# luvk1412/RoaringBitmap

Measured on AMD Instinct MI355X. Metric: wide-OR/pairwise-AND input GB/s + % of HBM peak at 1/2/4/8 MI355X, higher is better.
Workload: dtype u64; 1 GPU; C2: RoaringBitmap.and(x1, x2), two full 2^32-universe bitmaps of 65536 mixed array/bitmap/run containers each (configs[1]); per_rank=the whole pair, parallelism=key-range sharding over 1 GPU(s)

## Files before the change

### roaringbitmap_amd/csrc/pairwise.hip

```cpp
#include <algorithm>
#include <cstdio>
#include <cstdlib>

#include "kernels.hpp"
#include "wave.hpp"

namespace rbg {

__device__ __forceinline__ int pair_class(int op, int ka, int kb) {
  if (ka == kAbsent || kb == kAbsent) return 1;
  if (op == OP_AND && (ka == DK_A || kb == DK_A)) return 1;
  if (op == OP_ANDNOT && ka == DK_A) return 1;
  return 2;
}

__global__ __launch_bounds__(256) void k_plan_pairwise(int op, int key_lo, int key_hi, const uint32_t* __restrict__ koa,
                                                       const CDesc* __restrict__ da, const uint8_t* __restrict__ pa,
                                                       const uint32_t* __restrict__ kob,
                                                       const CDesc* __restrict__ db, const uint8_t* __restrict__ pb,
                                                       uint64_t* __restrict__ wg_epoch, uint32_t epoch,
                                                       PTask* __restrict__ tasks, uint32_t* __restrict__ n_tasks,
                                                       uint64_t* zlb, uint64_t* ztile, uint32_t* err) {
  plan_zero(zlb, ztile);
  const uint32_t k = blockIdx.x * blockDim.x + threadIdx.x;
// ... 37 lines not shown
    c = 18 + n / 300;
  }
  return kBalBins - 1 - min(c, kBalBins - 1);
}

template <int OP, int MODE>
__global__ __launch_bounds__(256) void k_plan_balanced(int key_lo, uint32_t nkeys, const uint32_t* __restrict__ koa,
                                                       const CDesc* __restrict__ da, const uint8_t* __restrict__ pa,
                                                       const uint32_t* __restrict__ kob,
                                                       const CDesc* __restrict__ db, const uint8_t* __restrict__ pb,
                                                       PTask* __restrict__ tasks, uint32_t* __restrict__ n_tasks,
                                                       OutCtx oc, uint32_t* __restrict__ task_card, uint64_t* zlb,
                                                       uint64_t* ztile) {
  __shared__ int hist[kBalBins];
  __shared__ int off[kBalBins];
  plan_zero(zlb, ztile);
  if (threadIdx.x < kBalBins) hist[threadIdx.x] = 0;
  __syncthreads();
  const uint32_t i = blockIdx.x * blockDim.x + threadIdx.x;
  PTask t;
  int bin = kBalBins - 1, rank = 0;
  if (i < nkeys) {
    const uint32_t k = (uint32_t)key_lo + i;
    resolve(koa, da, pa, k, t.slot_a, t.card_a, t.kind_a, t.nruns_a);
    resolve(kob, db, pb, k, t.slot_b, t.card_b, t.kind_b, t.nruns_b);
    t.key = (uint16_t)k;
    const bool ia = t.kind_a != kAbsent, ib = t.kind_b != kAbsent;
    const bool has = (OP == OP_OR || OP == OP_XOR) ? (ia || ib) : OP == OP_ANDNOT ? ia : (ia && ib);
    if (has) {
      bin = bal_bin<OP>(t);
    } else {
      t.kind_a = t.kind_b = kAbsent;
      if (MODE == 1) {
        task_card[i] = 0;
      } else {
        ORec r;
        r.off = 0;
        r.src = 0;
        r.idx = 0;
        r.card = 0;
        r.ser_len = 0;
        r.key = (uint16_t)k;
        r.kind = DK_A;
        r.keep = 0;
        oc.recs[i] = r;
      }
    }
    rank = atomicAdd(&hist[bin], 1);
  }
  __syncthreads();
  if (threadIdx.x == 0) {
    int run = 0;
    for (int b = 0; b < kBalBins; b++) {
      off[b] = run;
      run += hist[b];
    }
  }
  __syncthreads();
  if (i < nkeys) {
    const uint32_t m = min(256u, nkeys - blockIdx.x * 256u);
    const uint32_t r = (uint32_t)(off[bin] + rank);
    tasks[blockIdx.x * 256u + (r + blockIdx.x) % m] = t;
  }
  if (blockIdx.x == 0 && threadIdx.x == 0) {
    n_tasks[0] = nkeys;
    n_tasks[1] = nkeys;
  }
}

constexpr int kWaves = 4;
constexpr int kWaveLds = 2558;
static_assert(kWaveLds >= 2048, "the 8 KiB bitmap map / staging area");


__device__ __forceinline__ void prio_hi() { __builtin_amdgcn_s_setprio(3); }
__device__ __forceinline__ void prio_lo() {
  const uint32_t tier = __builtin_amdgcn_readfirstlane((blockIdx.x * 4u) / gridDim.x) >> 1;
  if (tier == 0) __builtin_amdgcn_s_setprio(0);
  else __builtin_amdgcn_s_setprio(1);
}

template <int OP, int MODE>
__device__ __forceinline__ void filter_task(uint32_t t, uint32_t key, int pcard, const uint8_t* pslot, int mkind,
                                            int mcard, const uint8_t* mslot, const OutCtx& oc, uint32_t* task_card,
                                            uint32_t* lds) {
  const int l = lane_id();
  const int nvec = (pcard + 7) >> 3;
  const uint4* pv = reinterpret_cast<const uint4*>(pslot) + l;
  uint4 v[8];
#pragma unroll
  for (int j = 0; j < 8; j++) v[j] = (64 * j + l < nvec) ? ld_in(pv + 64 * j) : make_uint4(0, 0, 0, 0);
  w_map_lds(mkind, mcard, mslot, lds);
  prio_lo();
  uint32_t hit[8];
  int cnt = 0;
#pragma unroll
  for (int j = 0; j < 8; j++) {
    hit[j] = 0;
    if (512 * j < pcard) {
      const int first = 8 * (64 * j + l);
      const uint32_t w[4] = {v[j].x, v[j].y, v[j].z, v[j].w};
      uint32_t h = 0;
#pragma unroll
      for (int i = 0; i < 8; i++) {
        const uint32_t wi = w[i >> 1];
        const uint32_t word = lds[(i & 1) ? bfe_hi_word(wi) : bfe_lo_word(wi)];
        h |= bit_at(word, (i & 1) ? (wi >> 16) : wi) << i;
      }
      if (OP == OP_ANDNOT) h = ~h & 0xFFu;
      const int rem = pcard - first;
      hit[j] = rem >= 8 ? h : h & ((1u << max(rem, 0)) - 1u);
      cnt += __popc(hit[j]);
    }
  }
  if (MODE == 1) {
    const int c = wave_sum_i(cnt);
    if (l == 0) task_card[t] = (uint32_t)c;
    return;
  }
  uint16_t* st = reinterpret_cast<uint16_t*>(lds);
  const uint32_t ctot = uni((uint32_t)wave_sum_i(cnt));
  const bool dummies = ctot <= 4096u - 64u;
  const uint32_t dummy = ctot + (uint32_t)l;
  wsync();
  int base = 0;
#pragma unroll
  for (int j = 0; j < 8; j += 2) {
    if (512 * j >= pcard) break;
    int tot;
    const int ex = wave_excl(__popc(hit[j]) | (__popc(hit[j + 1]) << 16), &tot);
    int q0 = base + (ex & 0xFFFF);
    int q1 = base + (tot & 0xFFFF) + (ex >> 16);
#pragma unroll
    for (int h = 0; h < 2; h++) {
      const uint32_t hj = hit[j + h];
      int q = h == 0 ? q0 : q1;
      const uint32_t w[4] = {v[j + h].x, v[j + h].y, v[j + h].z, v[j + h].w};
#pragma unroll
      for (int i = 0; i < 8; i++) {
        const uint32_t keep = (hj >> i) & 1u;
        const uint16_t val = (uint16_t)((w[i >> 1] >> ((i & 1) * 16)) & 0xFFFF);
        if (dummies) st[keep ? (uint32_t)q : dummy] = val;
        else if (keep) st[q] = val;
        q += (int)keep;
      }
    }
    base += (tot & 0xFFFF) + (tot >> 16);
  }
  const int c = (int)ctot;
  wsync();
  uint8_t* slot = oc.scratch + (size_t)t * kSlotBytes;
  const uint4* sv = reinterpret_cast<const uint4*>(lds);
  uint4* dv = reinterpret_cast<uint4*>(slot);
  for (int k = l; k < (2 * c + 15) >> 4; k += 64) dv[k] = sv[k];
  w_place(t, c > 0, slot, false, lds, 2u * (uint32_t)c, (uint32_t)c, key, DK_A, oc);
}

template <int OP, int MODE>
__device__ __forceinline__ void filter_class_task(uint32_t t, const PTask& tk, const uint8_t* pa, const uint8_t* pb,
                                                  const OutCtx& oc, uint32_t* task_card, uint32_t* lds) {
  const int ka = tk.kind_a, kb = tk.kind_b;
  if (ka == kAbsent || kb == kAbsent) {
    if (MODE == 0) {
      const bool from_a = ka != kAbsent;
      const int kind = from_a ? ka : kb;
      const uint32_t card = from_a ? tk.card_a : tk.card_b;
      const uint32_t nr = from_a ? tk.nruns_a : tk.nruns_b;
      const uint8_t* src = (from_a ? pa + tk.slot_a : pb + tk.slot_b) + (kind == DK_R ? 2 : 0);
      const uint32_t len = kind == DK_A ? 2 * card : kind == DK_B ? 8192u : 2 + 4 * nr;
      w_place(t, true, src, false, lds, len, card, tk.key, kind, oc);
    }
    return;
  }
  const int ca = (int)tk.card_a, cb = (int)tk.card_b;
  const uint8_t* sa = pa + tk.slot_a;
  const uint8_t* sb = pb + tk.slot_b;
  if (ka == DK_A && (OP == OP_ANDNOT || kb != DK_A || ca <= cb))
    filter_task<OP, MODE>(t, tk.key, ca, sa, kb, cb, sb, oc, task_card, lds);
  else
    filter_task<OP, MODE>(t, tk.key, cb, sb, ka, ca, sa, oc, task_card, lds);
}

constexpr uint32_t kRunSentinel = 0xFFFEFFFFu;
template <bool EMIT>
__device__ __forceinline__ void rr_merge(const uint32_t* lds, int na, int nb, int d0, int d1, int& cnt, int& card,
                                         uint32_t* out) {
  const uint32_t* al = lds;
  const uint32_t* bl = lds + na + 1;
  int lo = max(0, d0 - nb), hi = min(d0, na);
  while (lo < hi) {
    const int m = (lo + hi) >> 1;
    if ((al[m] >> 16) <= (bl[d0 - m - 1] >> 16)) lo = m + 1;
    else hi = m;
  }
  int i = lo, j = d0 - lo;
  uint32_t a = al[i], b = bl[j];
  uint32_t an = al[min(i + 1, na)], bn = bl[min(j + 1, nb)];
  for (int d = d0; d < d1; d++) {
    const uint32_t as = a & 0xFFFF, ae = a >> 16, bs = b & 0xFFFF, be = b >> 16;
    const uint32_t s0 = max(as, bs), e0 = min(ae, be);
    const bool ov = s0 <= e0;
    if (EMIT && ov) out[cnt] = s0 | ((e0 - s0) << 16);
    cnt += ov ? 1 : 0;
    card += ov ? (int)(e0 - s0 + 1) : 0;
    const bool adv = ae <= be;
    i = adv ? min(i + 1, na) : i;
    j = adv ? j : min(j + 1, nb);
    const uint32_t nx = adv ? al[min(i + 1, na)] : bl[min(j + 1, nb)];
    b = adv ? b : bn;
    bn = adv ? bn : nx;
    a = adv ? an : a;
    an = adv ? nx : an;
  }
}

__device__ __forceinline__ void run_vec_to_lds(const uint4 v, int q, int n, uint32_t* dst) {
  const uint32_t u[4] = {v.x, v.y, v.z, v.w};
#pragma unroll
  for (int c = 0; c < 4; c++) {
    const int r = 4 * q + c - 1;
    if (r >= 0 && r < n) dst[r] = (u[c] & 0xFFFF) | (min((u[c] & 0xFFFF) + (u[c] >> 16), 65535u) << 16);
  }
}

__device__ __forceinline__ void runs_to_lds2(const uint8_t* sa, int na, uint32_t* da, const uint8_t* sb, int nb,
                                             uint32_t* db) {
  constexpr int R = 4;
  const int l = lane_id();
  const int nva = (na + 4) >> 2, nvb = (nb + 4) >> 2;
  const uint4* a4 = reinterpret_cast<const uint4*>(sa);
  const uint4* b4 = reinterpret_cast<const uint4*>(sb);
#pragma unroll 1
  for (int j0 = 0; 64 * j0 < max(nva, nvb); j0 += R) {
    uint4 va[R], vb[R];
#pragma unroll
    for (int j = 0; j < R; j++) {
      const int q = 64 * (j0 + j) + l;
      va[j] = q < nva ? ld_in(a4 + q) : make_uint4(0, 0, 0, 0);
      vb[j] = q < nvb ? ld_in(b4 + q) : make_uint4(0, 0, 0, 0);
    }
#pragma unroll
    for (int j = 0; j < R; j++) {
      const int q = 64 * (j0 + j) + l;
      run_vec_to_lds(va[j], q, na, da);
      run_vec_to_lds(vb[j], q, nb, db);
    }
  }
}

template <int MODE>
__device__ __forceinline__ bool rr_and_task(uint32_t t, const PTask& tk, const uint8_t* pa, const uint8_t* pb,
                                            const OutCtx& oc, uint32_t* task_card, uint32_t* lds) {
  const int na = tk.nruns_a, nb = tk.nruns_b;
  if (na + nb + 2 > kWaveLds) return false;
  const int l = lane_id();
  wsync();
  runs_to_lds2(pa + tk.slot_a, na, lds, pb + tk.slot_b, nb, lds + na + 1);
  if (l == 0) {
    lds[na] = kRunSentinel;
    lds[na + 1 + nb] = kRunSentinel;
  }
  prio_lo();
  wsync();
  const int d0 = (l * (na + nb)) >> 6, d1 = ((l + 1) * (na + nb)) >> 6;
  int cnt = 0, card = 0;
  rr_merge<false>(lds, na, nb, d0, d1, cnt, card, nullptr);
  const int c = (int)uni((uint32_t)wave_sum_i(card));
  if (MODE == 1) {
    if (l == 0) task_card[t] = (uint32_t)c;
    return true;
  }
  if (c == 0) {
    w_place(t, false, nullptr, true, lds, 0, 0, tk.key, DK_A, oc);
    return true;
  }
  int nr;
  const int off = wave_excl(cnt, &nr);
  nr = (int)uni((uint32_t)nr);
  if (eff(c, nr) != DK_R) return false;
  uint8_t* slot = oc.scratch + (size_t)t * kSlotBytes;
  int cnt2 = 0, card2 = 0;
  rr_merge<true>(lds, na, nb, d0, d1, cnt2, card2, reinterpret_cast<uint32_t*>(slot + 4) + off);
  if (l == 0) *reinterpret_cast<uint16_t*>(slot + 2) = (uint16_t)nr;
  w_place(t, true, slot + 2, false, lds, 2u + 4u * (uint32_t)nr, (uint32_t)c, tk.key, DK_R, oc);
  return true;
}

template <int OP, int MODE>
__device__ __forceinline__ void bitmap_class_task(uint32_t t, const PTask& tk, const uint8_t* pa, const uint8_t* pb,
                                                  const OutCtx& oc, uint32_t* task_card, uint32_t* lds) {
  const int ka = tk.kind_a, kb = tk.kind_b;
  const int ca = (int)tk.card_a, cb = (int)tk.card_b;
  if (OP == OP_AND && ka == DK_R && kb == DK_R && rr_and_task<MODE>(t, tk, pa, pb, oc, task_card, lds)) return;
  WCtr x;
  w_materialize(CDesc{tk.slot_a, tk.card_a, tk.key, (uint8_t)ka, 0}, pa, lds, x);
  w_combine<OP>(CDesc{tk.slot_b, tk.card_b, tk.key, (uint8_t)kb, 0}, pb, lds, x);
  prio_lo();
  const int c = w_card(x);
  if (MODE == 1) {
    if (lane_id() == 0) task_card[t] = (uint32_t)c;
    return;
  }
  if (c == 0) {
    w_place(t, false, nullptr, true, lds, 0, 0, tk.key, DK_A, oc);
    return;
  }
  const bool use_eff = pairwise_needs_runs(OP, ka, ca, kb, cb);
  const int kind = use_eff ? eff(c, w_runs(x)) : pairwise_kind(OP, ka, kb, c);
  if (kind == DK_B) {
    uint8_t* slot = oc.scratch + (size_t)t * kSlotBytes;
    w_store_bitmap(slot, x);
    w_place(t, true, slot, false, lds, 8192, (uint32_t)c, tk.key, DK_B, oc);
    return;
  }
  uint32_t len;
  if (kind == DK_A) len = w_stage(DK_A, x, c, lds);
  else len = 2u + 4u * (uint32_t)w_stage_runs(x, lds);
  w_place(t, true, nullptr, true, lds, len, (uint32_t)c, tk.key, kind, oc);
}


template <int OP>
__device__ __forceinline__ bool has_task(const PTask& t) {
  const bool ia = t.kind_a != kAbsent, ib = t.kind_b != kAbsent;
  if (OP == OP_OR || OP == OP_XOR) return ia || ib;
  if (OP == OP_ANDNOT) return ia;
  return ia && ib;
}

template <int OP, int MODE>
__device__ __forceinline__ void any_task(uint32_t t, const PTask& tk, const uint8_t* pa, const uint8_t* pb,
                                         const OutCtx& oc, uint32_t* task_card, uint32_t* lds) {
  prio_hi();
  if (pair_class(OP, tk.kind_a, tk.kind_b) == 1)
    filter_class_task<OP, MODE>(t, tk, pa, pb, oc, task_card, lds);
  else
    bitmap_class_task<OP, MODE>(t, tk, pa, pb, oc, task_card, lds);
}

template <int OP, int MODE, bool DIRECT>
__global__ __launch_bounds__(256, 4) void k_pair_wave(const PTask* __restrict__ tasks,
                                                      const uint32_t* __restrict__ n_tasks, const uint8_t* pa,
                                                      const uint8_t* pb, OutCtx oc, uint32_t* __restrict__ task_card,
                                                      PwDirect dsrc) {
  __shared__ __align__(16) uint32_t lds_all[kWaves][kWaveLds];
  if (DIRECT) {
    plan_zero(dsrc.zlb, dsrc.ztile);
    if (blockIdx.x == 0 && threadIdx.x == 0) dsrc.n_tasks_out[0] = dsrc.n_tasks_write;
  }
  const uint32_t nt = DIRECT ? dsrc.nkeys : uni(*n_tasks);
  const int w = threadIdx.x >> 6;
  uint32_t* lds = lds_all[w];
  const uint32_t stride = gridDim.x * kWaves;
  const uint32_t t0 = uni(blockIdx.x * kWaves + w);
  if (t0 >= nt) return;
  uint32_t t = t0;
  if (DIRECT) {
    const uint32_t per = (((nt + stride - 1) / stride) + 3) & ~3u;
    PTask* mine = const_cast<PTask*>(tasks) + (size_t)t0 * per;
    const int l = lane_id();
    for (uint32_t k0 = 0; k0 < per; k0 += 64) {
      const uint32_t k = k0 + (uint32_t)l, tk = t0 + k * stride;
      if (k < per && tk < nt) {
        const uint32_t key = (uint32_t)dsrc.key_lo + tk;
        PTask r;
        resolve(dsrc.koa, dsrc.da, pa, key, r.slot_a, r.card_a, r.kind_a, r.nruns_a);
        resolve(dsrc.kob, dsrc.db, pb, key, r.slot_b, r.card_b, r.kind_b, r.nruns_b);
        r.key = (uint16_t)key;
        mine[k] = r;
      }
    }
    asm volatile("s_waitcnt vmcnt(0)" ::: "memory");
    uint32_t k = 0;
    PTask cur = load_task(mine, 0);
    for (;;) {
      const uint32_t tn = t + stride;
      PTask nxt;
      if (tn < nt) nxt = load_task(mine, k + 1);
      if (has_task<OP>(cur)) {
// ... 136 lines not shown
```

### roaringbitmap_amd/csrc/wave.hpp

```cpp
#pragma once
#include "device.hpp"

namespace rbg {

constexpr int WL = 64;

__device__ __forceinline__ int lane_id() { return threadIdx.x & 63; }
__device__ __forceinline__ uint32_t uni(uint32_t x) { return __builtin_amdgcn_readfirstlane(x); }
__device__ __forceinline__ uint64_t uni64(uint64_t x) {
  return ((uint64_t)(uint32_t)__builtin_amdgcn_readfirstlane((uint32_t)(x >> 32)) << 32) |
         (uint64_t)(uint32_t)__builtin_amdgcn_readfirstlane((uint32_t)x);
}

__device__ __forceinline__ uint4 ld_in(const uint4* p) {
  typedef unsigned int v4u __attribute__((ext_vector_type(4)));
  const v4u v = __builtin_nontemporal_load(reinterpret_cast<const v4u*>(p));
  return make_uint4(v.x, v.y, v.z, v.w);
}

__device__ __forceinline__ uint32_t bfe_lo_word(uint32_t w) {
  uint32_t r;
  asm("v_bfe_u32 %0, %1, 5, 11" : "=v"(r) : "v"(w));
  return r;
}
__device__ __forceinline__ uint32_t bfe_hi_word(uint32_t w) {
  uint32_t r;
  asm("v_bfe_u32 %0, %1, 21, 11" : "=v"(r) : "v"(w));
  return r;
}
__device__ __forceinline__ uint32_t bit_at(uint32_t word, uint32_t bit) {
  uint32_t r;
  asm("v_bfe_u32 %0, %1, %2, 1" : "=v"(r) : "v"(word), "v"(bit));
  return r;
}

__device__ __forceinline__ void wsync() {
  __builtin_amdgcn_fence(__ATOMIC_RELEASE, "wavefront");
  __builtin_amdgcn_wave_barrier();
  __builtin_amdgcn_fence(__ATOMIC_ACQUIRE, "wavefront");
}

__device__ __forceinline__ int wave_sum_i(int v) { return lane63(dpp_incl_scan(v)); }
__device__ __forceinline__ int wave_excl(int v, int* tot) {
  const int s = dpp_incl_scan(v);
  *tot = lane63(s);
  return s - v;
}

struct WCtr {
  uint64_t w[16];
};

__device__ __forceinline__ void w_zero(WCtr& x) {
#pragma unroll
  for (int k = 0; k < 16; k++) x.w[k] = 0;
}
__device__ __forceinline__ void w_ones(WCtr& x) {
#pragma unroll
  for (int k = 0; k < 16; k++) x.w[k] = ~0ULL;
}

__device__ __forceinline__ void w_load_bitmap(const uint8_t* p, WCtr& x) {
  const uint4* q = reinterpret_cast<const uint4*>(p) + lane_id();
#pragma unroll
  for (int i = 0; i < 8; i++) {
    const uint4 v = ld_in(q + 64 * i);
    x.w[2 * i] = (uint64_t)v.x | ((uint64_t)v.y << 32);
    x.w[2 * i + 1] = (uint64_t)v.z | ((uint64_t)v.w << 32);
  }
}
__device__ __forceinline__ uint64_t wrange(int k, int lo, int hi) {
  const int w = 128 * (k >> 1) + 2 * lane_id() + (k & 1);
  const int b0 = 64 * w, b1 = b0 + 63;
  if (b1 < lo || b0 > hi) return 0ull;
  uint64_t m = ~0ull;
  if (lo > b0) m &= ~0ull << (lo - b0);
  if (hi < b1) m &= ~0ull >> (b1 - hi);
  return m;
}

__device__ __forceinline__ void w_read_lds(const uint32_t* lds, WCtr& x) {
  const uint4* q = reinterpret_cast<const uint4*>(lds) + lane_id();
#pragma unroll
  for (int i = 0; i < 8; i++) {
    const uint4 v = q[64 * i];
    x.w[2 * i] = (uint64_t)v.x | ((uint64_t)v.y << 32);
    x.w[2 * i + 1] = (uint64_t)v.z | ((uint64_t)v.w << 32);
  }
}
__device__ __forceinline__ void w_write_lds(uint32_t* lds, const WCtr& x) {
  uint4* q = reinterpret_cast<uint4*>(lds) + lane_id();
#pragma unroll
  for (int i = 0; i < 8; i++)
    q[64 * i] = make_uint4((uint32_t)x.w[2 * i], (uint32_t)(x.w[2 * i] >> 32), (uint32_t)x.w[2 * i + 1],
                           (uint32_t)(x.w[2 * i + 1] >> 32));
}
__device__ __forceinline__ void w_clear_lds(uint32_t* lds) {
  uint4* q = reinterpret_cast<uint4*>(lds) + lane_id();
#pragma unroll
  for (int i = 0; i < 8; i++) q[64 * i] = make_uint4(0, 0, 0, 0);
}

constexpr int kVecRound = 4;

template <int MODE>
__device__ __forceinline__ void scatter_vec_mask(uint32_t* lds, const uint4 v, uint32_t vm) {
  const uint32_t w[4] = {v.x, v.y, v.z, v.w};
#pragma unroll
  for (int i = 0; i < 8; i++) {
    const uint32_t wi = w[i >> 1];
    uint32_t* p = lds + ((i & 1) ? bfe_hi_word(wi) : bfe_lo_word(wi));
    const uint32_t m = ((vm >> i) & 1u) << (((i & 1) ? (wi >> 16) : wi) & 31u);
    if (MODE == 0) atomicOr(p, m);
    else atomicXor(p, m);
  }
}

template <int MODE>
__device__ __forceinline__ void scatter_vec(uint32_t* lds, const uint4 v, int base, int card) {
  const int rem = card - base;
  scatter_vec_mask<MODE>(lds, v, rem >= 8 ? 0xFFu : (1u << max(rem, 0)) - 1u);
}

template <int MODE>
__device__ __forceinline__ void scatter_vec_merged(uint32_t* lds, const uint4 v, int base, int card) {
  const uint32_t w[4] = {v.x, v.y, v.z, v.w};
  uint32_t cur = 0xFFFFFFFFu, mask = 0;
#pragma unroll
  for (int i = 0; i < 8; i++) {
    if (base + i < card) {
      const uint32_t x = (w[i >> 1] >> ((i & 1) * 16)) & 0xFFFF;
      if ((x >> 5) != cur) {
        if (mask) {
          if (MODE == 0) atomicOr(&lds[cur], mask);
          else atomicXor(&lds[cur], mask);
        }
        cur = x >> 5;
        mask = 0;
      }
      mask |= 1u << (x & 31);
    }
  }
  if (mask) {
    if (MODE == 0) atomicOr(&lds[cur], mask);
    else atomicXor(&lds[cur], mask);
  }
}

template <int MODE>
__device__ __forceinline__ void w_scatter_array(uint32_t* lds, const uint16_t* vals, int card) {
  const int nvec = (card + 7) >> 3;
  const uint4* v4 = reinterpret_cast<const uint4*>(vals);
  const int l = lane_id();
#pragma unroll 1
  for (int j0 = 0; 64 * j0 < nvec; j0 += kVecRound) {
    uint4 v[kVecRound];
#pragma unroll
    for (int j = 0; j < kVecRound; j++) {
      const int k = 64 * (j0 + j) + l;
      v[j] = k < nvec ? ld_in(v4 + k) : make_uint4(0, 0, 0, 0);
    }
#pragma unroll
    for (int j = 0; j < kVecRound; j++) {
      const int base = 8 * (64 * (j0 + j) + l);
      if (base >= card) break;
      scatter_vec<MODE>(lds, v[j], base, card);
    }
  }
}

__device__ __forceinline__ void toggle_vec(uint32_t* lds, const uint4 v, int r0, int nruns) {
  const uint32_t u[4] = {v.x, v.y, v.z, v.w};
#pragma unroll
  for (int c = 0; c < 4; c++) {
    const int r = r0 + c;
    if (r >= 0 && r < nruns) {
      const uint32_t s = u[c] & 0xFFFF, e1 = s + (u[c] >> 16) + 1;
      atomicXor(&lds[s >> 5], 1u << (s & 31));
      if (e1 < 65536) atomicXor(&lds[e1 >> 5], 1u << (e1 & 31));
    }
  }
}

__device__ __forceinline__ void w_toggle_runs(uint32_t* lds, const uint8_t* slot, int nruns, int j_first = 0) {
  const int nvec = (nruns + 4) >> 2;
  const uint4* v4 = reinterpret_cast<const uint4*>(slot);
  const int l = lane_id();
#pragma unroll 1
  for (int j0 = j_first; 64 * j0 < nvec; j0 += kVecRound) {
    uint4 v[kVecRound];
#pragma unroll
    for (int j = 0; j < kVecRound; j++) {
      const int k = 64 * (j0 + j) + l;
      v[j] = k < nvec ? ld_in(v4 + k) : make_uint4(0, 0, 0, 0);
    }
#pragma unroll
    for (int j = 0; j < kVecRound; j++) {
      const int r0 = 4 * (64 * (j0 + j) + l) - 1;
      if (r0 >= nruns) break;
      toggle_vec(lds, v[j], r0, nruns);
    }
  }
}

__device__ __forceinline__ uint64_t prefix_xor64(uint64_t x) {
  x ^= x << 1;
  x ^= x << 2;
  x ^= x << 4;
  x ^= x << 8;
  x ^= x << 16;
  x ^= x << 32;
  return x;
}

__device__ __forceinline__ void w_run_chunk(const uint32_t* lds, int i, uint32_t& carry, uint64_t& w0, uint64_t& w1) {
  const int l = lane_id();
  const uint4 v = reinterpret_cast<const uint4*>(lds)[64 * i + l];
  uint64_t a = prefix_xor64((uint64_t)v.x | ((uint64_t)v.y << 32));
  uint64_t b = prefix_xor64((uint64_t)v.z | ((uint64_t)v.w << 32));
  if (a >> 63) b = ~b;
  const uint64_t m = __ballot((b >> 63) != 0);
  const uint32_t pre = ((uint32_t)__popcll(m & ((1ULL << l) - 1)) & 1u) ^ carry;
  if (pre) {
    a = ~a;
    b = ~b;
  }
  carry ^= (uint32_t)__popcll(m) & 1u;
  w0 = a;
  w1 = b;
}

__device__ __forceinline__ void w_materialize(const CDesc& d, const uint8_t* payload, uint32_t* lds, WCtr& x) {
  const uint8_t* slot = payload + d.slot;
  if (d.kind == DK_B) {
    w_load_bitmap(slot, x);
    return;
  }
  wsync();
// ... 22 lines not shown
}
template <int OP>
__device__ __forceinline__ void w_combine(const CDesc& d, const uint8_t* payload, uint32_t* lds, WCtr& x) {
  const uint8_t* slot = payload + d.slot;
  if (d.kind == DK_R) {
    wsync();
    w_clear_lds(lds);
    wsync();
    const int nr = *reinterpret_cast<const uint16_t*>(slot + 2);
    w_toggle_runs(lds, slot, nr);
    wsync();
    uint32_t carry = 0;
#pragma unroll
    for (int i = 0; i < 8; i++) {
      uint64_t a, b;
      w_run_chunk(lds, i, carry, a, b);
      x.w[2 * i] = w_op<OP>(x.w[2 * i], a);
      x.w[2 * i + 1] = w_op<OP>(x.w[2 * i + 1], b);
    }
    return;
  }
  if (d.kind == DK_B) {
    const uint4* g = reinterpret_cast<const uint4*>(slot) + lane_id();
#pragma unroll
    for (int i = 0; i < 8; i++) {
      const uint4 v = ld_in(g + 64 * i);
      x.w[2 * i] = w_op<OP>(x.w[2 * i], (uint64_t)v.x | ((uint64_t)v.y << 32));
      x.w[2 * i + 1] = w_op<OP>(x.w[2 * i + 1], (uint64_t)v.z | ((uint64_t)v.w << 32));
    }
    return;
  }
  wsync();
  w_clear_lds(lds);
  wsync();
  w_scatter_array<0>(lds, reinterpret_cast<const uint16_t*>(slot), (int)d.card);
  wsync();
  const uint4* q = reinterpret_cast<const uint4*>(lds) + lane_id();
#pragma unroll
  for (int i = 0; i < 8; i++) {
    const uint4 v = q[64 * i];
    x.w[2 * i] = w_op<OP>(x.w[2 * i], (uint64_t)v.x | ((uint64_t)v.y << 32));
    x.w[2 * i + 1] = w_op<OP>(x.w[2 * i + 1], (uint64_t)v.z | ((uint64_t)v.w << 32));
  }
}

__device__ __forceinline__ int w_card(const WCtr& x) {
  int c = 0;
#pragma unroll
  for (int k = 0; k < 16; k++) c += __popcll(x.w[k]);
  return (int)__builtin_amdgcn_readfirstlane((uint32_t)wave_sum_i(c));
}

template <int I>
__device__ __forceinline__ void w_chunk_edges(const WCtr& x, uint64_t& s0, uint64_t& s1, uint64_t& e0, uint64_t& e1) {
  const int l = lane_id();
  const uint64_t w0 = x.w[2 * I], w1 = x.w[2 * I + 1];
  const uint32_t top1 = from_prev_lane((uint32_t)(w1 >> 63));
  const uint32_t pchunk = I > 0 ? lane63u((uint32_t)(x.w[2 * (I > 0 ? I - 1 : 0) + 1] >> 63)) : 0u;
  const uint64_t prev0 = (l == 0) ? pchunk : top1;
  const uint32_t bot0 = from_next_lane((uint32_t)(w0 & 1));
  const uint32_t nchunk = I < 7 ? lane0u((uint32_t)(x.w[2 * (I < 7 ? I + 1 : 7)] & 1)) : 0u;
  const uint64_t next1 = (l == 63) ? nchunk : bot0;
  s0 = w0 & ~((w0 << 1) | prev0);
  s1 = w1 & ~((w1 << 1) | (w0 >> 63));
  e0 = w0 & ~((w0 >> 1) | ((w1 & 1) << 63));
  e1 = w1 & ~((w1 >> 1) | (next1 << 63));
}

template <int I>
__device__ __forceinline__ int w_runs_acc(const WCtr& x) {
  uint64_t s0, s1, e0, e1;
  w_chunk_edges<I>(x, s0, s1, e0, e1);
  return __popcll(s0) + __popcll(s1) + (I < 7 ? w_runs_acc<(I < 7 ? I + 1 : 7)>(x) : 0);
}

__device__ __forceinline__ int w_runs(const WCtr& x) {
  const int c = w_runs_acc<0>(x);
  return (int)__builtin_amdgcn_readfirstlane((uint32_t)wave_sum_i(c));
}

__device__ __forceinline__ int w_stage_runs(const WCtr& x, uint32_t* lds);

__device__ __forceinline__ uint32_t w_stage(int kind, const WCtr& x, int card, uint32_t* lds) {
  const int l = lane_id();
  if (kind == DK_B) {
    wsync();
    w_write_lds(lds, x);
    wsync();
    return 8192;
  }
  uint16_t* st = reinterpret_cast<uint16_t*>(lds);
  if (kind == DK_A) {
    wsync();
    int base = 0;
#pragma unroll
    for (int i = 0; i < 8; i++) {
      uint64_t v0 = x.w[2 * i], v1 = x.w[2 * i + 1];
      const int c0 = __popcll(v0);
      int tot;
      int p0 = base + wave_excl(c0 + __popcll(v1), &tot);
      int p1 = p0 + c0;
      const int wb = (128 * i + 2 * l) * 64;
      while (v0 | v1) {
        if (v0) {
          st[p0++] = (uint16_t)(wb + __builtin_ctzll(v0));
          v0 &= v0 - 1;
        }
        if (v1) {
          st[p1++] = (uint16_t)(wb + 64 + __builtin_ctzll(v1));
          v1 &= v1 - 1;
        }
      }
      base += tot;
    }
    wsync();
    return 2u * (uint32_t)card;
  }
  return 2u + 4u * (uint32_t)w_stage_runs(x, lds);
}

__device__ __forceinline__ int lower_bound_u16(const uint16_t* keys, int n, uint32_t k) {
  int lo = 0, hi = n;
  while (lo < hi) {
    const int mid = (lo + hi) >> 1;
    if (keys[mid] < k) lo = mid + 1;
    else hi = mid;
  }
  return lo;
}

__device__ __forceinline__ void plan_zero(uint64_t* lb_header, uint64_t* tile_status) {
  if (blockIdx.x != 0) return;
  if (lb_header && threadIdx.x < 32) lb_header[threadIdx.x] = 0;
  if (tile_status) {
    for (uint32_t i = threadIdx.x; i < (uint32_t)kMaxTiles; i += blockDim.x) tile_status[i] = 0;
    for (uint32_t i = threadIdx.x; i < (uint32_t)kMaxAggTiles; i += blockDim.x) tile_status[2 * kMaxTiles + i] = 0;
  }
}

__device__ __forceinline__ void resolve(const uint32_t* key_off, const CDesc* desc, const uint8_t* payload, uint32_t k,
                                        uint64_t& slot, uint32_t& card, uint8_t& kind, uint16_t& nruns) {
  const uint32_t p = key_off[k];
  if (key_off[k + 1] > p) {
    const CDesc d = desc[p];
    slot = d.slot;
    card = d.card;
    kind = d.kind;
    nruns = d.kind == DK_R ? *reinterpret_cast<const uint16_t*>(payload + d.slot + 2) : 0;
  } else {
    slot = 0;
    card = 0;
    kind = kAbsent;
    nruns = 0;
  }
}

__device__ __forceinline__ PTask load_task(const PTask* tasks, uint32_t t) {
  typedef const __attribute__((address_space(4))) uint64_t* CU64;
  const CU64 q = reinterpret_cast<CU64>(reinterpret_cast<uintptr_t>(tasks + t));
  union {
    uint64_t u[4];
    PTask p;
  } r;
#pragma unroll
  for (int i = 0; i < 4; i++) r.u[i] = q[i];
  return r.p;
}

__device__ __forceinline__ void plan_emit(int f, const PTask& t, uint64_t* wg_epoch, uint32_t epoch, PTask* tasks,
                                          uint32_t* n_tasks, uint32_t* err) {
  __shared__ int wt[4];
  __shared__ int wb[4];
  int tot;
  const int lane_pre = wave_excl(f, &tot);
  if ((threadIdx.x & 63) == 0) wt[threadIdx.x >> 6] = tot;
  __syncthreads();
  const int cnt = wt[0] + wt[1] + wt[2] + wt[3];
  if (threadIdx.x == 0)
    __hip_atomic_store(wg_epoch + blockIdx.x, ((uint64_t)epoch << 32) | (uint32_t)cnt, __ATOMIC_RELAXED,
                       __HIP_MEMORY_SCOPE_AGENT);
  uint32_t c = 0;
  if (threadIdx.x < blockIdx.x) {
    uint64_t v;
    uint32_t spins = 0;
    while (((v = __hip_atomic_load(wg_epoch + threadIdx.x, __ATOMIC_RELAXED, __HIP_MEMORY_SCOPE_AGENT)) >> 32) !=
           epoch) {
      if (++spins > (1u << 22)) {
        atomicOr(err, 1u);
        break;
      }
      __builtin_amdgcn_s_sleep(1);
    }
    c = (uint32_t)v;
  }
  const int sw = wave_sum_i((int)c);
  if ((threadIdx.x & 63) == 0) wb[threadIdx.x >> 6] = sw;
  __syncthreads();
  const uint32_t base = (uint32_t)(wb[0] + wb[1] + wb[2] + wb[3]);
  int wpre = 0;
  for (int i = 0; i < (int)(threadIdx.x >> 6); i++) wpre += wt[i];
  if (f) tasks[base + wpre + lane_pre] = t;
  if (blockIdx.x == gridDim.x - 1 && threadIdx.x == 0) *n_tasks = base + cnt;
}

__device__ __forceinline__ void plan_count(int f, uint32_t* wg_count) {
  __shared__ int wc[4];
  const uint64_t m = __ballot(f);
  if ((threadIdx.x & 63) == 0) wc[threadIdx.x >> 6] = __popcll(m);
  lds_barrier();
  if (threadIdx.x == 0) wg_count[blockIdx.x] = (uint32_t)(wc[0] + wc[1] + wc[2] + wc[3]);
}

__device__ __forceinline__ void w_store_bitmap(uint8_t* p, const WCtr& x) {
  uint4* q = reinterpret_cast<uint4*>(p) + lane_id();
#pragma unroll
  for (int i = 0; i < 8; i++) {
    const uint4 v = make_uint4((uint32_t)x.w[2 * i], (uint32_t)(x.w[2 * i] >> 32), (uint32_t)x.w[2 * i + 1],
                               (uint32_t)(x.w[2 * i + 1] >> 32));
    *reinterpret_cast<uint4*>(q + 64 * i) = v;
  }
}

constexpr int kPre = 8;
struct WPre {
  uint4 v[kPre];
};

__device__ __forceinline__ int slot_nvec(int kind, int card, int nruns) {
  return kind == DK_A ? (2 * card + 15) >> 4 : kind == DK_B ? 512 : (nruns + 4) >> 2;
}

__device__ __forceinline__ void w_prefetch(const uint8_t* slot, int nvec, WPre& p) {
  const uint4* q = reinterpret_cast<const uint4*>(slot) + lane_id();
  const int l = lane_id();
#pragma unroll
  for (int j = 0; j < kPre; j++) p.v[j] = (64 * j + l < nvec) ? q[64 * j] : make_uint4(0, 0, 0, 0);
}

template <int MODE>
__device__ __forceinline__ void w_scatter_pre(uint32_t* lds, const WPre& p, int card) {
  const int l = lane_id();
#pragma unroll
  for (int j = 0; j < kPre; j++) {
    if (512 * j >= card) break;
    scatter_vec<MODE>(lds, p.v[j], 8 * (64 * j + l), card);
    __builtin_amdgcn_sched_barrier(0);
  }
}

__device__ __forceinline__ void w_toggle_pre(uint32_t* lds, const WPre& p, const uint8_t* slot, int nruns) {
  const int l = lane_id();
  const int nvec = (nruns + 4) >> 2;
#pragma unroll
  for (int j = 0; j < kPre; j++) {
    if (64 * j >= nvec) break;
    toggle_vec(lds, p.v[j], 4 * (64 * j + l) - 1, nruns);
    __builtin_amdgcn_sched_barrier(0);
  }
  if (nvec > 64 * kPre) w_toggle_runs(lds, slot, nruns, kPre);
}

__device__ __forceinline__ void pre_to_words(const WPre& p, WCtr& x) {
#pragma unroll
  for (int i = 0; i < 8; i++) {
    x.w[2 * i] = (uint64_t)p.v[i].x | ((uint64_t)p.v[i].y << 32);
    x.w[2 * i + 1] = (uint64_t)p.v[i].z | ((uint64_t)p.v[i].w << 32);
  }
}

__device__ __forceinline__ void w_materialize_pre(int kind, int card, int nruns, const WPre& p, const uint8_t* slot,
                                                  uint32_t* lds, WCtr& x) {
  if (kind == DK_B) {
    pre_to_words(p, x);
    return;
  }
  wsync();
  w_clear_lds(lds);
  wsync();
  if (kind == DK_A) {
    w_scatter_pre<0>(lds, p, card);
    wsync();
    w_read_lds(lds, x);
    return;
  }
  w_toggle_pre(lds, p, slot, nruns);
  wsync();
  uint32_t carry = 0;
#pragma unroll
  for (int i = 0; i < 8; i++) w_run_chunk(lds, i, carry, x.w[2 * i], x.w[2 * i + 1]);
}

template <int OP>
__device__ __forceinline__ void w_combine_pre(int kind, int card, int nruns, const WPre& p, const uint8_t* slot,
                                              uint32_t* lds, WCtr& x) {
  if (kind == DK_B) {
#pragma unroll
    for (int i = 0; i < 8; i++) {
      x.w[2 * i] = w_op<OP>(x.w[2 * i], (uint64_t)p.v[i].x | ((uint64_t)p.v[i].y << 32));
      x.w[2 * i + 1] = w_op<OP>(x.w[2 * i + 1], (uint64_t)p.v[i].z | ((uint64_t)p.v[i].w << 32));
    }
    return;
  }
  wsync();
  w_clear_lds(lds);
  wsync();
  if (kind == DK_A) {
    w_scatter_pre<0>(lds, p, card);
    wsync();
    const uint4* q = reinterpret_cast<const uint4*>(lds) + lane_id();
#pragma unroll
    for (int i = 0; i < 8; i++) {
      const uint4 v = q[64 * i];
      x.w[2 * i] = w_op<OP>(x.w[2 * i], (uint64_t)v.x | ((uint64_t)v.y << 32));
      x.w[2 * i + 1] = w_op<OP>(x.w[2 * i + 1], (uint64_t)v.z | ((uint64_t)v.w << 32));
    }
    return;
  }
  w_toggle_pre(lds, p, slot, nruns);
  wsync();
  uint32_t carry = 0;
#pragma unroll
  for (int i = 0; i < 8; i++) {
    uint64_t a, b;
    w_run_chunk(lds, i, carry, a, b);
    x.w[2 * i] = w_op<OP>(x.w[2 * i], a);
    x.w[2 * i + 1] = w_op<OP>(x.w[2 * i + 1], b);
  }
}

__device__ __forceinline__ void w_map_pre(int kind, int card, int nruns, const WPre& p, const uint8_t* slot,
                                          uint32_t* lds) {
  const int l = lane_id();
  uint4* q = reinterpret_cast<uint4*>(lds) + l;
  wsync();
  if (kind == DK_B) {
#pragma unroll
    for (int i = 0; i < 8; i++) q[64 * i] = p.v[i];
    wsync();
    return;
  }
  w_clear_lds(lds);
  wsync();
  if (kind == DK_A) {
    w_scatter_pre<0>(lds, p, card);
    wsync();
    return;
  }
  w_toggle_pre(lds, p, slot, nruns);
  wsync();
  uint32_t carry = 0;
#pragma unroll
  for (int i = 0; i < 8; i++) {
    uint64_t a, b;
    w_run_chunk(lds, i, carry, a, b);
    q[64 * i] = make_uint4((uint32_t)a, (uint32_t)(a >> 32), (uint32_t)b, (uint32_t)(b >> 32));
  }
  wsync();
}

typedef __attribute__((address_space(3))) void* lds_void_ptr;
typedef __attribute__((address_space(1))) void* global_void_ptr;
__device__ __forceinline__ void w_bitmap_to_lds_dma(const uint8_t* slot, uint32_t* lds) {
  const uint4* g = reinterpret_cast<const uint4*>(slot) + lane_id();
  asm volatile("s_waitcnt lgkmcnt(0)" ::: "memory");
#pragma unroll
  for (int i = 0; i < 8; i++)
    __builtin_amdgcn_global_load_lds((global_void_ptr)(g + 64 * i), (lds_void_ptr)(lds + 256 * i), 16, 0,
                                     2 );
  asm volatile("s_waitcnt vmcnt(0)" ::: "memory");
}

__device__ __forceinline__ void w_map_lds(int kind, int card, const uint8_t* slot, uint32_t* lds) {
  wsync();
  if (kind == DK_B) {
    w_bitmap_to_lds_dma(slot, lds);
    wsync();
    return;
  }
  const int l = lane_id();
  uint4* q = reinterpret_cast<uint4*>(lds) + l;
  w_clear_lds(lds);
  wsync();
  if (kind == DK_A) {
    w_scatter_array<0>(lds, reinterpret_cast<const uint16_t*>(slot), card);
    wsync();
    return;
  }
  w_toggle_runs(lds, slot, *reinterpret_cast<const uint16_t*>(slot + 2));
  wsync();
  uint32_t carry = 0;
#pragma unroll
  for (int i = 0; i < 8; i++) {
    uint64_t a, b;
    w_run_chunk(lds, i, carry, a, b);
    q[64 * i] = make_uint4((uint32_t)a, (uint32_t)(a >> 32), (uint32_t)b, (uint32_t)(b >> 32));
  }
  wsync();
}

constexpr int kProbeRound = 2;
template <bool INV, bool WRITE>
__device__ __forceinline__ int w_probe_array(const uint32_t* lds, const uint16_t* vals, int n, uint16_t* out) {
  const int l = lane_id();
  const uint4* v4 = reinterpret_cast<const uint4*>(vals);
  const int nvec = (n + 7) >> 3;
  int base = 0;
#pragma unroll 1
  for (int j0 = 0; 64 * j0 < nvec; j0 += kProbeRound) {
    uint4 v[kProbeRound];
#pragma unroll
    for (int j = 0; j < kProbeRound; j++) {
      const int k = 64 * (j0 + j) + l;
      v[j] = k < nvec ? v4[k] : make_uint4(0, 0, 0, 0);
    }
#pragma unroll
    for (int j = 0; j < kProbeRound; j++) {
      if (64 * (j0 + j) >= nvec) break;
      const int first = 8 * (64 * (j0 + j) + l);
      const uint32_t w[4] = {v[j].x, v[j].y, v[j].z, v[j].w};
      uint32_t hit = 0;
#pragma unroll
      for (int i = 0; i < 8; i++) {
        const uint32_t x = (w[i >> 1] >> ((i & 1) * 16)) & 0xFFFF;
        const uint32_t m = (lds[x >> 5] >> (x & 31)) & 1u;
        hit |= ((INV ? (m ^ 1u) : m) & (first + i < n ? 1u : 0u)) << i;
      }
      int tot;
      int q = base + wave_excl(__popc(hit), &tot);
      if (WRITE) {
#pragma unroll
        for (int i = 0; i < 8; i++)
          if ((hit >> i) & 1u) out[q++] = (uint16_t)((w[i >> 1] >> ((i & 1) * 16)) & 0xFFFF);
      }
      base += tot;
    }
  }
  return (int)uni((uint32_t)base);
}

template <bool INV, bool WRITE>
__device__ __forceinline__ int w_probe_pre(const uint32_t* lds, const WPre& p, int n, uint16_t* out) {
  const int l = lane_id();
  int base = 0;
#pragma unroll
  for (int j = 0; j < kPre; j++) {
    if (512 * j >= n) break;
    const int first = 8 * (64 * j + l);
    const uint32_t w[4] = {p.v[j].x, p.v[j].y, p.v[j].z, p.v[j].w};
    uint32_t hit = 0;
#pragma unroll
    for (int i = 0; i < 8; i++) {
      const uint32_t x = (w[i >> 1] >> ((i & 1) * 16)) & 0xFFFF;
      const uint32_t m = (lds[x >> 5] >> (x & 31)) & 1u;
      hit |= ((INV ? (m ^ 1u) : m) & (first + i < n ? 1u : 0u)) << i;
    }
    int tot;
    int q = base + wave_excl(__popc(hit), &tot);
    if (WRITE) {
#pragma unroll
      for (int i = 0; i < 8; i++)
        if ((hit >> i) & 1u) out[q++] = (uint16_t)((w[i >> 1] >> ((i & 1) * 16)) & 0xFFFF);
    }
    base += tot;
  }
  return (int)uni((uint32_t)base);
}

template <int I, int CAP = 2047>
__device__ __forceinline__ int w_stage_runs_chunk(const WCtr& x, uint16_t* st, int base, int base_e) {
  const int l = lane_id();
  uint64_t s0, s1, e0, e1;
  w_chunk_edges<I>(x, s0, s1, e0, e1);
  const int cs0 = __popcll(s0), ce0 = __popcll(e0);
  const int cs = cs0 + __popcll(s1), ce = ce0 + __popcll(e1);
  int tot;
  const int packed = wave_excl(cs | (ce << 16), &tot);
  const int wb = (128 * I + 2 * l) * 64;
  int ps0 = base + (packed & 0xFFFF), ps1 = ps0 + cs0;
  int pe0 = base_e + (packed >> 16), pe1 = pe0 + ce0;
  while (s0 | s1 | e0 | e1) {
    if (s0) {
      if (ps0 < CAP) st[1 + 2 * ps0] = (uint16_t)(wb + __builtin_ctzll(s0));
      ps0++;
      s0 &= s0 - 1;
    }
    if (s1) {
      if (ps1 < CAP) st[1 + 2 * ps1] = (uint16_t)(wb + 64 + __builtin_ctzll(s1));
      ps1++;
      s1 &= s1 - 1;
    }
    if (e0) {
      if (pe0 < CAP) st[2 + 2 * pe0] = (uint16_t)(wb + __builtin_ctzll(e0));
      pe0++;
      e0 &= e0 - 1;
    }
    if (e1) {
      if (pe1 < CAP) st[2 + 2 * pe1] = (uint16_t)(wb + 64 + __builtin_ctzll(e1));
      pe1++;
      e1 &= e1 - 1;
    }
  }
  const int nb = base + (tot & 0xFFFF), nbe = base_e + (tot >> 16);
  if (I < 7) return w_stage_runs_chunk<(I < 7 ? I + 1 : 7), CAP>(x, st, nb, nbe);
  return nb;
}

__device__ __forceinline__ int w_stage_runs(const WCtr& x, uint32_t* lds) {
  uint16_t* st = reinterpret_cast<uint16_t*>(lds);
  wsync();
  const int nr = (int)uni((uint32_t)w_stage_runs_chunk<0>(x, st, 0, 0));
  const int ns = nr < 2047 ? nr : 2047;
  wsync();
  for (int k = lane_id(); k < ns; k += 64) st[2 + 2 * k] = (uint16_t)(st[2 + 2 * k] - st[1 + 2 * k]);
  if (lane_id() == 0) st[0] = (uint16_t)ns;
  wsync();
  return nr;
}

template <int G>
__device__ __forceinline__ void copy_lds_to_global(uint8_t* dst, const uint32_t* lds, uint32_t n, int lane) {
  const uintptr_t d = reinterpret_cast<uintptr_t>(dst);
  uint32_t head = (uint32_t)((16 - (d & 15)) & 15);
  if (head > n) head = n;
  const uint16_t* l16 = reinterpret_cast<const uint16_t*>(lds);
  uint16_t* d16 = reinterpret_cast<uint16_t*>(dst);
  for (uint32_t i = lane; i < head / 2; i += G) d16[i] = l16[i];
  const uint32_t body = (n - head) & ~15u;
  uint4* dv = reinterpret_cast<uint4*>(dst + head);
  const uint32_t sh = head & 3;
  const uint32_t w0 = head >> 2;
  for (uint32_t c = lane; c < body / 16; c += G) {
    const uint32_t* q = lds + w0 + 4 * c;
    if (sh == 0) {
      dv[c] = make_uint4(q[0], q[1], q[2], q[3]);
    } else {
      const uint32_t a0 = q[0], a1 = q[1], a2 = q[2], a3 = q[3], a4 = q[4];
      dv[c] = make_uint4(__builtin_amdgcn_alignbyte(a1, a0, 2), __builtin_amdgcn_alignbyte(a2, a1, 2),
                         __builtin_amdgcn_alignbyte(a3, a2, 2), __builtin_amdgcn_alignbyte(a4, a3, 2));
    }
  }
  const uint32_t done = head + body;
  for (uint32_t i = done / 2 + lane; i < n / 2; i += G) d16[i] = l16[i];
}

struct Prefix {
  uint32_t idx;
  uint64_t off;
};

__device__ __forceinline__ uint64_t lb_pack(uint64_t st, uint64_t run, uint64_t cnt, uint64_t bytes) {
  return (st << 62) | (run << 61) | (cnt << 44) | bytes;
}

// ... 265 lines not shown
```

Before: 2397 GB/s.

## Issue container loads early and build LDS maps from prefetched registers

Bitmap-class pairwise tasks now issue the global loads for both non-bitmap operands (or the other operand alongside the bitmap load) before building their LDS maps. Each map is then built from the registers already loaded, and the array/run combine reads straight from LDS. This removes serial load-then-scatter latency per container and passes run counts directly instead of rereading them from the slot header. It also adds lane_here(), an opaque lane index that blocks compiler rematerialisation, which may raise register pressure. The now-unused WPre helpers are removed.

```diff
diff --git a/roaringbitmap_amd/csrc/pairwise.hip b/roaringbitmap_amd/csrc/pairwise.hip
--- a/roaringbitmap_amd/csrc/pairwise.hip
+++ b/roaringbitmap_amd/csrc/pairwise.hip
@@ -143,15 +143,15 @@
 
 template <int OP, int MODE>
 __device__ __forceinline__ void filter_task(uint32_t t, uint32_t key, int pcard, const uint8_t* pslot, int mkind,
-                                            int mcard, const uint8_t* mslot, const OutCtx& oc, uint32_t* task_card,
+                                            int mn, const uint8_t* mslot, const OutCtx& oc, uint32_t* task_card,
                                             uint32_t* lds) {
-  const int l = lane_id();
+  const int l = lane_here();
   const int nvec = (pcard + 7) >> 3;
   const uint4* pv = reinterpret_cast<const uint4*>(pslot) + l;
   uint4 v[8];
 #pragma unroll
   for (int j = 0; j < 8; j++) v[j] = (64 * j + l < nvec) ? ld_in(pv + 64 * j) : make_uint4(0, 0, 0, 0);
-  w_map_lds(mkind, mcard, mslot, lds);
+  w_map_lds(mkind, mn, mslot, lds);
   prio_lo();
   uint32_t hit[8];
   int cnt = 0;
@@ -237,9 +237,9 @@
   const uint8_t* sa = pa + tk.slot_a;
   const uint8_t* sb = pb + tk.slot_b;
   if (ka == DK_A && (OP == OP_ANDNOT || kb != DK_A || ca <= cb))
-    filter_task<OP, MODE>(t, tk.key, ca, sa, kb, cb, sb, oc, task_card, lds);
+    filter_task<OP, MODE>(t, tk.key, ca, sa, kb, kb == DK_R ? (int)tk.nruns_b : cb, sb, oc, task_card, lds);
   else
-    filter_task<OP, MODE>(t, tk.key, cb, sb, ka, ca, sa, oc, task_card, lds);
+    filter_task<OP, MODE>(t, tk.key, cb, sb, ka, ka == DK_R ? (int)tk.nruns_a : ca, sa, oc, task_card, lds);
 }
 
 constexpr uint32_t kRunSentinel = 0xFFFEFFFFu;
@@ -353,9 +353,31 @@
   const int ka = tk.kind_a, kb = tk.kind_b;
   const int ca = (int)tk.card_a, cb = (int)tk.card_b;
   if (OP == OP_AND && ka == DK_R && kb == DK_R && rr_and_task<MODE>(t, tk, pa, pb, oc, task_card, lds)) return;
+  const uint8_t* sa = pa + tk.slot_a;
+  const uint8_t* sb = pb + tk.slot_b;
+  const int na = ka == DK_R ? (int)tk.nruns_a : ca, nb = kb == DK_R ? (int)tk.nruns_b : cb;
   WCtr x;
-  w_materialize(CDesc{tk.slot_a, tk.card_a, tk.key, (uint8_t)ka, 0}, pa, lds, x);
-  w_combine<OP>(CDesc{tk.slot_b, tk.card_b, tk.key, (uint8_t)kb, 0}, pb, lds, x);
+  if (ka == DK_B && kb == DK_B) {
+    w_materialize(CDesc{tk.slot_a, tk.card_a, tk.key, (uint8_t)ka, 0}, pa, lds, x);
+    w_combine<OP>(CDesc{tk.slot_b, tk.card_b, tk.key, (uint8_t)kb, 0}, pb, lds, x);
+  } else if (ka == DK_B || kb == DK_B) {
+    const bool swap = kb == DK_B;
+    const int ko = swap ? ka : kb, no = swap ? na : nb;
+    const uint8_t* so = swap ? sa : sb;
+    WRound r;
+    w_request(so, slot_nvec(ko, no), r);
+    w_load_bitmap(swap ? sb : sa, x);
+    w_build_lds(ko, lds, so, no, r);
+    w_combine_lds<OP>(ko, lds, x, swap);
+  } else {
+    WRound ra, rb;
+    w_request(sa, slot_nvec(ka, na), ra);
+    w_request(sb, slot_nvec(kb, nb), rb);
+    w_build_lds(ka, lds, sa, na, ra);
+    w_take_lds(ka, lds, x);
+    w_build_lds(kb, lds, sb, nb, rb);
+    w_combine_lds<OP>(kb, lds, x, false);
+  }
   prio_lo();
   const int c = w_card(x);
   if (MODE == 1) {
diff --git a/roaringbitmap_amd/csrc/wave.hpp b/roaringbitmap_amd/csrc/wave.hpp
--- a/roaringbitmap_amd/csrc/wave.hpp
+++ b/roaringbitmap_amd/csrc/wave.hpp
@@ -6,6 +6,11 @@
 constexpr int WL = 64;
 
 __device__ __forceinline__ int lane_id() { return threadIdx.x & 63; }
+__device__ __forceinline__ int lane_here() {
+  int l = threadIdx.x & 63;
+  asm volatile("" : "+v"(l));
+  return l;
+}
 __device__ __forceinline__ uint32_t uni(uint32_t x) { return __builtin_amdgcn_readfirstlane(x); }
 __device__ __forceinline__ uint64_t uni64(uint64_t x) {
   return ((uint64_t)(uint32_t)__builtin_amdgcn_readfirstlane((uint32_t)(x >> 32)) << 32) |
@@ -148,12 +153,12 @@
 }
 
 template <int MODE>
-__device__ __forceinline__ void w_scatter_array(uint32_t* lds, const uint16_t* vals, int card) {
+__device__ __forceinline__ void w_scatter_array(uint32_t* lds, const uint16_t* vals, int card, int j_first = 0) {
   const int nvec = (card + 7) >> 3;
   const uint4* v4 = reinterpret_cast<const uint4*>(vals);
   const int l = lane_id();
 #pragma unroll 1
-  for (int j0 = 0; 64 * j0 < nvec; j0 += kVecRound) {
+  for (int j0 = j_first; 64 * j0 < nvec; j0 += kVecRound) {
     uint4 v[kVecRound];
 #pragma unroll
     for (int j = 0; j < kVecRound; j++) {
@@ -342,7 +347,7 @@
 __device__ __forceinline__ int w_stage_runs(const WCtr& x, uint32_t* lds);
 
 __device__ __forceinline__ uint32_t w_stage(int kind, const WCtr& x, int card, uint32_t* lds) {
-  const int l = lane_id();
+  const int l = lane_here();
   if (kind == DK_B) {
     wsync();
     w_write_lds(lds, x);
@@ -481,143 +486,6 @@
   }
 }
 
-constexpr int kPre = 8;
-struct WPre {
-  uint4 v[kPre];
-};
-
-__device__ __forceinline__ int slot_nvec(int kind, int card, int nruns) {
-  return kind == DK_A ? (2 * card + 15) >> 4 : kind == DK_B ? 512 : (nruns + 4) >> 2;
-}
-
-__device__ __forceinline__ void w_prefetch(const uint8_t* slot, int nvec, WPre& p) {
-  const uint4* q = reinterpret_cast<const uint4*>(slot) + lane_id();
-  const int l = lane_id();
-#pragma unroll
-  for (int j = 0; j < kPre; j++) p.v[j] = (64 * j + l < nvec) ? q[64 * j] : make_uint4(0, 0, 0, 0);
-}
-
-template <int MODE>
-__device__ __forceinline__ void w_scatter_pre(uint32_t* lds, const WPre& p, int card) {
-  const int l = lane_id();
-#pragma unroll
-  for (int j = 0; j < kPre; j++) {
-    if (512 * j >= card) break;
-    scatter_vec<MODE>(lds, p.v[j], 8 * (64 * j + l), card);
-    __builtin_amdgcn_sched_barrier(0);
-  }
-}
-
-__device__ __forceinline__ void w_toggle_pre(uint32_t* lds, const WPre& p, const uint8_t* slot, int nruns) {
-  const int l = lane_id();
-  const int nvec = (nruns + 4) >> 2;
-#pragma unroll
-  for (int j = 0; j < kPre; j++) {
-    if (64 * j >= nvec) break;
-    toggle_vec(lds, p.v[j], 4 * (64 * j + l) - 1, nruns);
-    __builtin_amdgcn_sched_barrier(0);
-  }
-  if (nvec > 64 * kPre) w_toggle_runs(lds, slot, nruns, kPre);
-}
-
-__device__ __forceinline__ void pre_to_words(const WPre& p, WCtr& x) {
-#pragma unroll
-  for (int i = 0; i < 8; i++) {
-    x.w[2 * i] = (uint64_t)p.v[i].x | ((uint64_t)p.v[i].y << 32);
-    x.w[2 * i + 1] = (uint64_t)p.v[i].z | ((uint64_t)p.v[i].w << 32);
-  }
-}
-
-__device__ __forceinline__ void w_materialize_pre(int kind, int card, int nruns, const WPre& p, const uint8_t* slot,
-                                                  uint32_t* lds, WCtr& x) {
-  if (kind == DK_B) {
-    pre_to_words(p, x);
-    return;
-  }
-  wsync();
-  w_clear_lds(lds);
-  wsync();
-  if (kind == DK_A) {
-    w_scatter_pre<0>(lds, p, card);
-    wsync();
-    w_read_lds(lds, x);
-    return;
-  }
-  w_toggle_pre(lds, p, slot, nruns);
-  wsync();
-  uint32_t carry = 0;
-#pragma unroll
-  for (int i = 0; i < 8; i++) w_run_chunk(lds, i, carry, x.w[2 * i], x.w[2 * i + 1]);
-}
-
-template <int OP>
-__device__ __forceinline__ void w_combine_pre(int kind, int card, int nruns, const WPre& p, const uint8_t* slot,
-                                              uint32_t* lds, WCtr& x) {
-  if (kind == DK_B) {
-#pragma unroll
-    for (int i = 0; i < 8; i++) {
-      x.w[2 * i] = w_op<OP>(x.w[2 * i], (uint64_t)p.v[i].x | ((uint64_t)p.v[i].y << 32));
-      x.w[2 * i + 1] = w_op<OP>(x.w[2 * i + 1], (uint64_t)p.v[i].z | ((uint64_t)p.v[i].w << 32));
-    }
-    return;
-  }
-  wsync();
-  w_clear_lds(lds);
-  wsync();
-  if (kind == DK_A) {
-    w_scatter_pre<0>(lds, p, card);
-    wsync();
-    const uint4* q = reinterpret_cast<const uint4*>(lds) + lane_id();
-#pragma unroll
-    for (int i = 0; i < 8; i++) {
-      const uint4 v = q[64 * i];
-      x.w[2 * i] = w_op<OP>(x.w[2 * i], (uint64_t)v.x | ((uint64_t)v.y << 32));
-      x.w[2 * i + 1] = w_op<OP>(x.w[2 * i + 1], (uint64_t)v.z | ((uint64_t)v.w << 32));
-    }
-    return;
-  }
-  w_toggle_pre(lds, p, slot, nruns);
-  wsync();
-  uint32_t carry = 0;
-#pragma unroll
-  for (int i = 0; i < 8; i++) {
-    uint64_t a, b;
-    w_run_chunk(lds, i, carry, a, b);
-    x.w[2 * i] = w_op<OP>(x.w[2 * i], a);
-    x.w[2 * i + 1] = w_op<OP>(x.w[2 * i + 1], b);
-  }
-}
-
-__device__ __forceinline__ void w_map_pre(int kind, int card, int nruns, const WPre& p, const uint8_t* slot,
-                                          uint32_t* lds) {
-  const int l = lane_id();
-  uint4* q = reinterpret_cast<uint4*>(lds) + l;
-  wsync();
-  if (kind == DK_B) {
-#pragma unroll
-    for (int i = 0; i < 8; i++) q[64 * i] = p.v[i];
-    wsync();
-    return;
-  }
-  w_clear_lds(lds);
-  wsync();
-  if (kind == DK_A) {
-    w_scatter_pre<0>(lds, p, card);
-    wsync();
-    return;
-  }
-  w_toggle_pre(lds, p, slot, nruns);
-  wsync();
-  uint32_t carry = 0;
-#pragma unroll
-  for (int i = 0; i < 8; i++) {
-    uint64_t a, b;
-    w_run_chunk(lds, i, carry, a, b);
-    q[64 * i] = make_uint4((uint32_t)a, (uint32_t)(a >> 32), (uint32_t)b, (uint32_t)(b >> 32));
-  }
-  wsync();
-}
-
 typedef __attribute__((address_space(3))) void* lds_void_ptr;
 typedef __attribute__((address_space(1))) void* global_void_ptr;
 __device__ __forceinline__ void w_bitmap_to_lds_dma(const uint8_t* slot, uint32_t* lds) {
@@ -630,24 +498,92 @@
   asm volatile("s_waitcnt vmcnt(0)" ::: "memory");
 }
 
-__device__ __forceinline__ void w_map_lds(int kind, int card, const uint8_t* slot, uint32_t* lds) {
-  wsync();
+struct WRound {
+  uint4 v[kVecRound];
+};
+__device__ __forceinline__ int slot_nvec(int kind, int n) { return kind == DK_A ? (n + 7) >> 3 : (n + 4) >> 2; }
+
+__device__ __forceinline__ void w_request(const uint8_t* slot, int nvec, WRound& r) {
+  const int l = lane_here();
+  const uint4* q = reinterpret_cast<const uint4*>(slot) + l;
+#pragma unroll
+  for (int j = 0; j < kVecRound; j++) r.v[j] = (64 * j + l < nvec) ? ld_in(q + 64 * j) : make_uint4(0, 0, 0, 0);
+}
+
+__device__ __forceinline__ void w_build_lds(int kind, uint32_t* lds, const uint8_t* slot, int n, const WRound& r) {
+  const int l = lane_here();
+  wsync();
+  w_clear_lds(lds);
+  wsync();
+  if (kind == DK_A) {
+#pragma unroll
+    for (int j = 0; j < kVecRound; j++) {
+      const int base = 8 * (64 * j + l);
+      if (base >= n) break;
+      scatter_vec<0>(lds, r.v[j], base, n);
+    }
+    if (n > 512 * kVecRound) w_scatter_array<0>(lds, reinterpret_cast<const uint16_t*>(slot), n, kVecRound);
+  } else {
+#pragma unroll
+    for (int j = 0; j < kVecRound; j++) {
+      const int r0 = 4 * (64 * j + l) - 1;
+      if (r0 >= n) break;
+      toggle_vec(lds, r.v[j], r0, n);
+    }
+    if (slot_nvec(DK_R, n) > 64 * kVecRound) w_toggle_runs(lds, slot, n, kVecRound);
+  }
+  wsync();
+}
+
+__device__ __forceinline__ void w_take_lds(int kind, const uint32_t* lds, WCtr& x) {
+  if (kind == DK_A) {
+    w_read_lds(lds, x);
+    return;
+  }
+  uint32_t carry = 0;
+#pragma unroll
+  for (int i = 0; i < 8; i++) w_run_chunk(lds, i, carry, x.w[2 * i], x.w[2 * i + 1]);
+}
+
+template <int OP>
+__device__ __forceinline__ uint64_t w_op_sw(uint64_t x, uint64_t y, bool swap) {
+  if (OP == 3 && swap) return y & ~x;
+  return w_op<OP>(x, y);
+}
+template <int OP>
+__device__ __forceinline__ void w_combine_lds(int kind, const uint32_t* lds, WCtr& x, bool swap) {
+  if (kind == DK_R) {
+    uint32_t carry = 0;
+#pragma unroll
+    for (int i = 0; i < 8; i++) {
+      uint64_t a, b;
+      w_run_chunk(lds, i, carry, a, b);
+      x.w[2 * i] = w_op_sw<OP>(x.w[2 * i], a, swap);
+      x.w[2 * i + 1] = w_op_sw<OP>(x.w[2 * i + 1], b, swap);
+    }
+    return;
+  }
+  const uint4* q = reinterpret_cast<const uint4*>(lds) + lane_here();
+#pragma unroll
+  for (int i = 0; i < 8; i++) {
+    const uint4 v = q[64 * i];
+    x.w[2 * i] = w_op_sw<OP>(x.w[2 * i], (uint64_t)v.x | ((uint64_t)v.y << 32), swap);
+    x.w[2 * i + 1] = w_op_sw<OP>(x.w[2 * i + 1], (uint64_t)v.z | ((uint64_t)v.w << 32), swap);
+  }
+}
+
+__device__ __forceinline__ void w_map_lds(int kind, int n, const uint8_t* slot, uint32_t* lds) {
   if (kind == DK_B) {
+    wsync();
     w_bitmap_to_lds_dma(slot, lds);
     wsync();
     return;
   }
-  const int l = lane_id();
-  uint4* q = reinterpret_cast<uint4*>(lds) + l;
-  w_clear_lds(lds);
-  wsync();
-  if (kind == DK_A) {
-    w_scatter_array<0>(lds, reinterpret_cast<const uint16_t*>(slot), card);
-    wsync();
-    return;
-  }
-  w_toggle_runs(lds, slot, *reinterpret_cast<const uint16_t*>(slot + 2));
-  wsync();
+  WRound r;
+  w_request(slot, slot_nvec(kind, n), r);
+  w_build_lds(kind, lds, slot, n, r);
+  if (kind == DK_A) return;
+  uint4* q = reinterpret_cast<uint4*>(lds) + lane_here();
   uint32_t carry = 0;
 #pragma unroll
   for (int i = 0; i < 8; i++) {
@@ -698,37 +634,9 @@
   return (int)uni((uint32_t)base);
 }
 
-template <bool INV, bool WRITE>
-__device__ __forceinline__ int w_probe_pre(const uint32_t* lds, const WPre& p, int n, uint16_t* out) {
-  const int l = lane_id();
-  int base = 0;
-#pragma unroll
-  for (int j = 0; j < kPre; j++) {
-    if (512 * j >= n) break;
-    const int first = 8 * (64 * j + l);
-    const uint32_t w[4] = {p.v[j].x, p.v[j].y, p.v[j].z, p.v[j].w};
-    uint32_t hit = 0;
-#pragma unroll
-    for (int i = 0; i < 8; i++) {
-      const uint32_t x = (w[i >> 1] >> ((i & 1) * 16)) & 0xFFFF;
-      const uint32_t m = (lds[x >> 5] >> (x & 31)) & 1u;
-      hit |= ((INV ? (m ^ 1u) : m) & (first + i < n ? 1u : 0u)) << i;
-    }
-    int tot;
-    int q = base + wave_excl(__popc(hit), &tot);
-    if (WRITE) {
-#pragma unroll
-      for (int i = 0; i < 8; i++)
-        if ((hit >> i) & 1u) out[q++] = (uint16_t)((w[i >> 1] >> ((i & 1) * 16)) & 0xFFFF);
-    }
-    base += tot;
-  }
-  return (int)uni((uint32_t)base);
-}
-
 template <int I, int CAP = 2047>
 __device__ __forceinline__ int w_stage_runs_chunk(const WCtr& x, uint16_t* st, int base, int base_e) {
-  const int l = lane_id();
+  const int l = lane_here();
   uint64_t s0, s1, e0, e1;
   w_chunk_edges<I>(x, s0, s1, e0, e1);
   const int cs0 = __popcll(s0), ce0 = __popcll(e0);
```

Result: slower. 2303 GB/s (-3.9%).
